# nikhilTkur/Multigrid_Nikhil_C-

Hardware: AMD Instinct MI355X
Metric: fine_grid_stencil_updates_per_sec (higher is better)
Workload: dtype f64

## Files before the change

### multigrid_nikhil_c-_amd/csrc/mgx.hip

```cpp

#include "../../include/mgx.h"
#include "mgx_bottom.hpp"
#include "mgx_kernels.hpp"
#include "mgx_launch.hpp"
#include "mgx_var.hpp"
#include "mgx_galerkin.hpp"
#include "mgx_opdep.hpp"
#include "mgx_cheby.hpp"
#include "mgx_line.hpp"
#include "mgx_small.hpp"
#include "mgx_krylov.hpp"
#include "mgx_dist_plan.hpp"

#include <chrono>
#include <unistd.h>
#include <cmath>
#include <cstdio>
#include <cstdlib>
#include <cstring>
#include <string>
#include <vector>

namespace {

using namespace mgx;

thread_local std::string g_create_error;

void log_runtime_libs(const char* where)
{
    if (env_int("MGX_LOG_RUNTIME_LIBS", 0) == 0) return;
    char buf[8192];
    if (mgx_runtime_libs(buf, sizeof buf) >= 0)
        std::fprintf(stderr, "[mgx] runtime libraries mapped at %s (pid %d):\n%s", where, (int)getpid(), buf);
}

struct Level {
    int L = 0, N = 0, rows = 0;
    long pitch = 0;
    size_t bytes = 0;
    bool f64 = true;
    void *u = nullptr, *b = nullptr, *tmp = nullptr, *r = nullptr;
    void* A[9] = {};
    void* J[9] = {};
    void* wt[8] = {nullptr, nullptr, nullptr, nullptr, nullptr, nullptr, nullptr, nullptr};
    bool nine = false;
// ... 197 lines not shown
    if (l.r) return MGX_OK;
    if (hipMalloc(&l.r, l.bytes) != hipSuccess) return s->fail(MGX_ERR_ALLOC, "hipMalloc failed for residual array");
    HIPCHK(s, hipMemsetAsync(l.r, 0, l.bytes, s->stream));
    return MGX_OK;
}

bool level_ok(const mgx_solver* s, int level)
{
    return level >= s->cfg.coarsest_level && level <= s->cfg.finest_level;
}

int copy_in(mgx_solver* s, Level& l, void* dst_grid, const void* src, size_t count)
{
    const size_t n = (size_t)l.N - 1;
    if (count != n * n) return s->fail(MGX_ERR_INVALID, "vector length must be n*n with n = 2^level - 1");
    const size_t es = l.esize();
    char* d = reinterpret_cast<char*>(dst_grid) + ((size_t)l.pitch + 1) * es;
    HIPCHK(s, hipMemcpy2DAsync(d, (size_t)l.pitch * es, src, n * es, n * es, n, hipMemcpyHostToDevice, s->stream));
    HIPCHK(s, hipStreamSynchronize(s->stream));
    return MGX_OK;
}

int copy_out(mgx_solver* s, Level& l, const void* src_grid, void* dst, size_t count)
{
    const size_t n = (size_t)l.N - 1;
    if (count != n * n) return s->fail(MGX_ERR_INVALID, "vector length must be n*n with n = 2^level - 1");
    const size_t es = l.esize();
    const char* p = reinterpret_cast<const char*>(src_grid) + ((size_t)l.pitch + 1) * es;
    HIPCHK(s, hipMemcpy2DAsync(dst, n * es, p, (size_t)l.pitch * es, n * es, n, hipMemcpyDeviceToHost, s->stream));
    HIPCHK(s, hipStreamSynchronize(s->stream));
    return MGX_OK;
}

inline bool tile_level(const mgx_solver* s, const Level& l) { return s->fuse.tile_max_n > 0 && l.N <= s->fuse.tile_max_n; }

BlockReq level_req(const mgx_solver* s, const Level& l, int mu, bool pre, int post, bool zero_in, int rpc)
{
    BlockReq q{s->cfg.smoother, l.f64, l.N, 0, l.rows, 1, l.N, mu, pre, post, zero_in};
    q.tile_points = (long)(s->fuse.tile_max_n - 1) * s->fuse.tile_max_n;
    q.rpc = rpc;
    return q;
}

int var_alloc_level(mgx_solver* s, Level& l)
{
    for (int q = 0; q < (l.nine ? 9 : 5); ++q)
        for (void** p : {&l.A[q], &l.J[q]}) {
            if (hipMalloc(p, l.bytes) != hipSuccess)
                return s->fail(MGX_ERR_ALLOC, q < 5 ? "hipMalloc failed for the operator's coefficient arrays"
                                                    : "hipMalloc failed for the nine-point operator's corner arrays");
            HIPCHK(s, hipMemsetAsync(*p, 0, l.bytes, s->stream));
        }
    return MGX_OK;
}

void gj_invert(mgx_solver* s, int NN)
{
    for (int k = 0; k < NN; ++k) {
        hipLaunchKernelGGL(k_gj_prow, dim3((NN + 255) / 256), dim3(256), 0, s->stream, s->var_M, s->var_inv, s->var_pm, s->var_pi, NN, k);
        hipLaunchKernelGGL(k_gj_elim, dim3(NN), dim3(256), 0, s->stream, s->var_M, s->var_inv, s->var_pm, s->var_pi, NN, k);
    }
}

void drop_graphs(mgx_solver* s)
{
    for (auto& g : s->graphs) if (g.exec) (void)hipGraphExecDestroy(g.exec);
// ... 876 lines not shown
    if (var && (cfg->dtype == MGX_DTYPE_MIXED || cfg->smoother == MGX_SMOOTHER_RBGS || cfg->arith != MGX_ARITH_SEPARATE || cfg->n_gpus > 1)) {
        g_create_error = cheby ? "MGX_SMOOTHER_CHEBYSHEV: dtype F64 or F32, arith SEPARATE, one GPU"
                       : galerkin ? "MGX_OPERATOR_GALERKIN: dtype F64 or F32, Jacobi or Chebyshev, arith SEPARATE, one GPU"
                                  : "MGX_OPERATOR_STENCIL5: dtype F64 or F32, Jacobi (MF:75-96) or Chebyshev, arith SEPARATE, one GPU";
        return MGX_ERR_INVALID;
    }
    if (galerkin && cfg->restrict_mode >= MGX_RESTRICT_INJECT) {
        g_create_error = "MGX_OPERATOR_GALERKIN: restrict_mode CONSISTENT or FW16 (R A P needs R = c P^T; injection has no variational meaning)";
        return MGX_ERR_INVALID;
    }
    if (cfg->restrict_mode >= MGX_RESTRICT_INJECT && (cfg->n_gpus > 1 || cfg->dtype == MGX_DTYPE_MIXED)) {
        g_create_error = "injection restriction (MF:122-130): single-GPU handles of dtype F64 or F32";
        return MGX_ERR_INVALID;
    }
    if (cfg->n_gpus > 1) return mgx_create_rank(cfg, -1, 1, nullptr, nullptr, out);
    log_runtime_libs("mgx_create");
    int ndev = 0;
    if (hipGetDeviceCount(&ndev) != hipSuccess || ndev <= 0 || cfg->device < 0 || cfg->device >= ndev) {
        g_create_error = "no usable HIP device (libmgx has no CPU fallback)";
        return MGX_ERR_NO_DEVICE;
    }
    if (hipSetDevice(cfg->device) != hipSuccess) { g_create_error = "hipSetDevice failed"; return MGX_ERR_HIP; }

    mgx_solver* s = new (std::nothrow) mgx_solver();
    if (!s) { g_create_error = "out of host memory"; return MGX_ERR_ALLOC; }
    s->cfg = *cfg;
    s->mixed = (cfg->dtype == MGX_DTYPE_MIXED);
    s->var = var;
    s->galerkin = galerkin;
    s->work_f64 = (cfg->dtype == MGX_DTYPE_F64);
    s->rows_per_chunk = env_int("MGX_ROWS", 0);
    s->fuse = fuse_cfg();
    s->fuse.arith = cfg->arith;
    s->fold = env_int("MGX_FOLD", 1);
    s->use_zero_in = env_int("MGX_ZERO_IN", 1);
    s->use_graph = env_int("MGX_GRAPH", 1);
    s->small_visit = env_int("MGX_SMALL_VISIT", 1);
    s->line_dirs = cfg->smoother == MGX_SMOOTHER_LINE_X ? 1 : cfg->smoother == MGX_SMOOTHER_LINE_Y ? 2 : cfg->smoother == MGX_SMOOTHER_LINE_ALT ? 3 : 0;
    int rc = MGX_OK;
    auto bail = [&](int code) { g_create_error = s->err; mgx_destroy(s); return code; };
    if (hipStreamCreate(&s->stream) != hipSuccess) { s->err = "hipStreamCreate failed"; return bail(MGX_ERR_HIP); }
    s->lv.resize(cfg->finest_level + 1);
    for (int l = cfg->coarsest_level; l <= cfg->finest_level; ++l)
        if ((rc = alloc_level(s, s->lv[l], l, s->work_f64)) != MGX_OK) return bail(rc);
    if (s->mixed && (rc = alloc_level(s, s->fine64, cfg->finest_level, true)) != MGX_OK) return bail(rc);
    if (var || cfg->restrict_mode >= MGX_RESTRICT_INJECT) {
        for (int l = cfg->coarsest_level + 1; l <= cfg->finest_level; ++l)
            if ((rc = ensure_r(s, s->lv[l])) != MGX_OK) return bail(rc);
    }
    if (galerkin && s->small_visit) {
        if (small_visit_prepare<double>() != hipSuccess || small_visit_prepare<float>() != hipSuccess) {
            s->err = "hipFuncSetAttribute failed for k_small_visit";
            return bail(MGX_ERR_HIP);
        }
    }
    if (var) {
        for (int l = cfg->coarsest_level; l <= cfg->finest_level; ++l) {
            s->lv[l].nine = galerkin && l < cfg->finest_level;
            if ((rc = var_alloc_level(s, s->lv[l])) != MGX_OK) return bail(rc);
            if (cheby) {
                Level& lv = s->lv[l];
                if (hipMalloc(&lv.cheb, lv.bytes) != hipSuccess) { s->err = "hipMalloc failed for the Chebyshev direction array"; return bail(MGX_ERR_ALLOC); }
                if (hipMemsetAsync(lv.cheb, 0, lv.bytes, s->stream) != hipSuccess) { s->err = "hipMemsetAsync failed"; return bail(MGX_ERR_HIP); }
            }
            if (line) {
                Level& lv = s->lv[l];
                lv.line_R = line_chunk_rows(lv.N, env_int("MGX_LINE_CHUNK", 0));
                std::vector<void**> arrays;
                for (int d = 0; d < 2; ++d)
                    if (s->line_dirs & (1 << d)) { arrays.push_back(&lv.line_m[d]); arrays.push_back(&lv.line_g[d]); }
                if ((s->line_dirs & 2) && line_chunks(lv.N, lv.line_R) > 1) { arrays.push_back(&lv.line_hf); arrays.push_back(&lv.line_hb); }
                for (void** p : arrays) {
                    if (hipMalloc(p, lv.bytes) != hipSuccess) { s->err = "hipMalloc failed for the line smoother's factor arrays"; return bail(MGX_ERR_ALLOC); }
                    if (hipMemsetAsync(*p, 0, lv.bytes, s->stream) != hipSuccess) { s->err = "hipMemsetAsync failed"; return bail(MGX_ERR_HIP); }
                }
            }
        }
        if (line && hipMalloc(&s->line_flag, sizeof(int)) != hipSuccess) { s->err = "hipMalloc failed for the line smoother's breakdown flag"; return bail(MGX_ERR_ALLOC); }
        if (cfg->bottom == MGX_BOTTOM_EXACT) {
            const size_t NN = (size_t)((1 << cfg->coarsest_level) - 1) * ((1 << cfg->coarsest_level) - 1);
            if (hipMalloc(&s->var_M, NN * NN * sizeof(double)) != hipSuccess || hipMalloc(&s->var_inv, NN * NN * sizeof(double)) != hipSuccess ||
                hipMalloc(&s->var_pm, NN * sizeof(double)) != hipSuccess || hipMalloc(&s->var_pi, NN * sizeof(double)) != hipSuccess) {
                s->err = "allocation of the coarsest operator's dense inverse failed";
                return bail(MGX_ERR_ALLOC);
            }
        }
    }
    s->mixed_fuse = env_int("MGX_MIXED_FUSE", 1);
    if (s->mixed && !s->mixed_fuse) { (void)hipFree(s->fine64.tmp); s->fine64.tmp = nullptr; }
    {
        const int N = 1 << cfg->finest_level;
        long cap = 0;
        for (int rpc : {s->rows_per_chunk, 1}) {
            cap = std::max(cap, sumsq_blocks<double>(N, N, rpc));
            cap = std::max(cap, sumsq_blocks<float>(N, N, rpc));
        }
        if (N <= s->fuse.tile_max_n) cap = std::max(cap, (long)((N + 31) / 32) * ((N + 39) / 40));
        s->partial_cap = cap + 8;
        if (hipMalloc(&s->partial, s->partial_cap * sizeof(double)) != hipSuccess ||
            hipMalloc(&s->sum_dev, sizeof(double)) != hipSuccess ||
            hipHostMalloc(&s->sum_host, sizeof(double)) != hipSuccess) {
            s->err = "allocation of reduction buffers failed";
            return bail(MGX_ERR_ALLOC);
        }
    }
    if (cfg->bottom == MGX_BOTTOM_EXACT && !var) {
        if (s->bottom.init((1 << cfg->coarsest_level) - 1) != hipSuccess) {
            s->err = "bottom solver allocation failed";
            return bail(MGX_ERR_ALLOC);
        }
    }
    if (hipStreamSynchronize(s->stream) != hipSuccess) { s->err = "device initialisation failed"; return bail(MGX_ERR_HIP); }
    *out = s;
    return MGX_OK;
}

int mgx_destroy(mgx_handle s)
{
    if (!s) return MGX_OK;
    if (s->dist) { dist_free(s->dist); s->dist = nullptr; }
    if (s->stream) (void)hipStreamSynchronize(s->stream);
    for (auto& l : s->lv) free_level(l);
    free_level(s->fine64);
    s->bottom.destroy();
    if (s->partial) (void)hipFree(s->partial);
    if (s->sum_dev) (void)hipFree(s->sum_dev);
    if (s->line_flag) (void)hipFree(s->line_flag);
    if (s->sum_host) (void)hipHostFree(s->sum_host);
    for (double* p : {s->var_M, s->var_inv, s->var_pm, s->var_pi}) if (p) (void)hipFree(p);
    s->kry.free();
// ... 690 lines not shown
    if (result_in_tmp) *result_in_tmp = flips & 1;
    return hipGetLastError() == hipSuccess ? MGX_OK : MGX_ERR_HIP;
}

int mgx_slab_jacobi(const mgx_slab* s, void* u, const void* b, void* tmp, int row_lo, int row_hi, int mu,
                    double omega, int shrink, int* result_in_tmp, void* stream)
{
    return slab_smooth(MGX_SMOOTHER_JACOBI, s, u, b, tmp, row_lo, row_hi, mu, omega, shrink, result_in_tmp, stream);
}

int mgx_slab_rbgs(const mgx_slab* s, void* u, const void* b, void* tmp, int row_lo, int row_hi, int mu,
                  int shrink, int* result_in_tmp, void* stream)
{
    return slab_smooth(MGX_SMOOTHER_RBGS, s, u, b, tmp, row_lo, row_hi, mu, 1.0, shrink, result_in_tmp, stream);
}

int mgx_slab_cycle(const mgx_slab* f, void* u, const void* b, void* tmp, int row_lo, int row_hi, int mu, double omega,
                   int smoother, const mgx_slab* c, const void* coarse_e, void* coarse_b, int crow_lo, int crow_hi,
                   int restrict_mode, int zero_in, double* scratch, double* sum_dev, int* result_in_tmp, void* stream)
{
    if (zero_in && coarse_e) return MGX_ERR_INVALID;
    if (smoother != MGX_SMOOTHER_JACOBI && smoother != MGX_SMOOTHER_RBGS) return MGX_ERR_INVALID;
    if (restrict_mode != MGX_RESTRICT_CONSISTENT && restrict_mode != MGX_RESTRICT_FW16) return MGX_ERR_INVALID;
    if (coarse_b && !((std::max(row_lo + f->row0, 1)) & 1)) return MGX_ERR_INVALID;
    if (slab_check(f) || !u || !b || !tmp || mu < 1 || mu > 64 || row_hi <= row_lo) return MGX_ERR_INVALID;
    if ((coarse_e || coarse_b) && (slab_check(c) || c->level != f->level - 1 || c->dtype != f->dtype)) return MGX_ERR_INVALID;
    if (coarse_b && sum_dev) return MGX_ERR_INVALID;
    if (sum_dev && !scratch) return MGX_ERR_INVALID;
    if (coarse_b && (crow_lo < 0 || crow_hi > c->rows || crow_hi < crow_lo)) return MGX_ERR_INVALID;
    const int N = 1 << f->level;
    if (row_lo < 0 || row_hi > f->rows || row_lo + f->row0 < 1 || row_hi + f->row0 > N) return MGX_ERR_INVALID;
    FuseCfg fc = fuse_cfg();
    fc.arith = f->arith;
    const int post = coarse_b ? 1 : (sum_dev ? 2 : 0);
    BlockReq q = slab_req(*f, smoother, row_lo, row_hi, mu, coarse_e != nullptr, post, zero_in != 0);
    q.tile_points = env_int("MGX_SLAB_TILE_POINTS", 1 << 20);
    const long pitch = level_pitch(f->level, f->dtype);
    hipStream_t st = (hipStream_t)stream;
    int flips = 0;
    const int nb = with_kernel_set(q.f64, smoother, f->arith, [&](auto k) {
        using K = decltype(k);
        using T = typename K::T;
        return fold_block<T, K::SM, K::AR>(fc, q, (T*)u, (const T*)b, (T*)tmp, pitch, omega, c, (const T*)coarse_e,
                                           (T*)coarse_b, nullptr, crow_lo, crow_hi, restrict_mode, scratch, st, &flips);
    });
    if (nb < 0) return MGX_ERR_INVALID;
    if (post == 2) hipLaunchKernelGGL(k_reduce_partials, dim3(1), dim3(kReduceThreads), 0, st, scratch, nb, sum_dev);
    if (result_in_tmp) *result_in_tmp = flips & 1;
    return hipGetLastError() == hipSuccess ? MGX_OK : MGX_ERR_HIP;
}

int mgx_slab_restrict(const mgx_slab* f, const void* u, const void* b, const mgx_slab* c, void* cb, void* zero_u,
                      int crow_lo, int crow_hi, int restrict_mode, int fused, void* stream)
{
    if (slab_check(f) || slab_check(c) || !b || !cb || (fused && !u)) return MGX_ERR_INVALID;
    if (restrict_mode != MGX_RESTRICT_CONSISTENT && restrict_mode != MGX_RESTRICT_FW16) return MGX_ERR_INVALID;
    if (c->level != f->level - 1 || c->dtype != f->dtype) return MGX_ERR_INVALID;
    const int N = 1 << f->level;
    const long pitch = level_pitch(f->level, f->dtype), cpitch = level_pitch(c->level, c->dtype);
    const int off = 2 * c->row0 - f->row0;
    const int halo = fused ? 2 : 1;
    if (crow_lo < 0 || crow_hi > c->rows || crow_lo + c->row0 < 1 || crow_hi + c->row0 > N / 2) return MGX_ERR_INVALID;
    if (crow_hi > crow_lo && (2 * crow_lo + off - halo < 0 || 2 * (crow_hi - 1) + off + halo > f->rows - 1)) return MGX_ERR_INVALID;
    const int rpc = env_int("MGX_ROWS", 0);
    if (f->dtype == MGX_DTYPE_F64)
        launch_restrict<double>((const double*)u, (const double*)b, (double*)cb, (double*)zero_u, N, pitch, cpitch,
// ... 231 lines not shown
```

### multigrid_nikhil_c-_amd/csrc/mgx_bottom.hpp

```cpp
#pragma once

#include <hip/hip_runtime.h>
#include <cmath>
#include <type_traits>
#include <vector>

#include "mgx_phase_trace.hpp"

#ifndef MGX_DST_DEEP
#define MGX_DST_DEEP 32
#endif

namespace mgx {

constexpr unsigned kDstOob = 0xFFFFFF00u;
__device__ __forceinline__ __amdgpu_buffer_rsrc_t dst_rsrc(const void* p, unsigned bytes)
{
    return __builtin_amdgcn_make_buffer_rsrc(const_cast<void*>(p), 0, (int)bytes, 0x00020000);
}
template <typename E> __device__ __forceinline__ double dst_load(__amdgpu_buffer_rsrc_t r, unsigned voff, unsigned soff)
{
    if constexpr (sizeof(E) == 8) {
        const auto t = __builtin_amdgcn_raw_buffer_load_b64(r, voff, soff, 0);
        return __hiloint2double(t[1], t[0]);
    } else {
        return (double)__int_as_float(__builtin_amdgcn_raw_buffer_load_b32(r, voff, soff, 0));
    }
}
template <typename E, int D>
__device__ __forceinline__ void dst_batch(double (&x)[D], __amdgpu_buffer_rsrc_t r, unsigned voff, unsigned rowbytes, int k0, int n)
{
    const unsigned last = (unsigned)(n - 1) * rowbytes;
    unsigned off = (unsigned)k0 * rowbytes;
#pragma unroll
    for (int q = 0; q < D; ++q, off += rowbytes) x[q] = dst_load<E>(r, voff, min(off, last));
}
template <int CNT, int D> __device__ __forceinline__ void dst_chain(double& acc, const double* m, const double (&x)[D])
{
#pragma unroll
    for (int q = 0; q < CNT; ++q) acc += m[q] * x[q];
}
template <int D> __device__ __forceinline__ void dst_chain_last(double& acc, const double* m, const double (&x)[D], int rem)
{
    if (rem == D - 1) {
        dst_chain<D - 1>(acc, m, x);
    } else {
#pragma unroll
        for (int q = 0; q < D; ++q)
            if (q < rem) acc += m[q] * x[q];
    }
}
template <int D, typename Load, typename Before, typename Stamp>
__device__ __forceinline__ double dst_dot(const double* m, int n, double (&xa)[D], Load load, Before before_last, Stamp landed)
{
    double xb[D];
    double acc = 0.0;
    int k = 0;
    for (;;) {
        if (k + D >= n) { before_last(); landed(xa[D - 1]); dst_chain_last<D>(acc, m + k, xa, n - k); break; }
        load(xb, k + D);
        landed(xa[D - 1]);
        dst_chain<D, D>(acc, m + k, xa);
        k += D;
        if (k + D >= n) { before_last(); landed(xb[D - 1]); dst_chain_last<D>(acc, m + k, xb, n - k); break; }
        load(xa, k + D);
        landed(xb[D - 1]);
        dst_chain<D, D>(acc, m + k, xb);
        k += D;
    }
    return acc;
}

template <typename T, bool FIRST>
__global__ void __launch_bounds__(256)
k_dst_pair(const double* __restrict__ S, const void* __restrict__ Xv, void* __restrict__ Ov, const double* __restrict__ s,
           int n, long gpitch)
{
    using E = std::conditional_t<FIRST, T, double>;
    __shared__ double srow[256], prow[256];
    MGX_PHASE_BEGIN();
    const int j = threadIdx.x;
    const int i = blockIdx.x;
    const bool live = j < n;
    constexpr int kDeep = MGX_DST_DEEP;
    const unsigned srb = (unsigned)n * 8u, xrb = FIRST ? (unsigned)gpitch * (unsigned)sizeof(T) : srb;
    const char* xp = static_cast<const char*>(Xv) + (FIRST ? (gpitch + 1) * (long)sizeof(T) : 0L);
    const __amdgpu_buffer_rsrc_t rs = dst_rsrc(S, (unsigned)n * srb);
    const __amdgpu_buffer_rsrc_t rx = dst_rsrc(xp, (unsigned)(n - 1) * xrb + (unsigned)n * (unsigned)sizeof(E));
    const unsigned vs = live ? (unsigned)j * 8u : kDstOob, vx = live ? (unsigned)j * (unsigned)sizeof(E) : kDstOob;
    auto landed = [&](const double& v) { MGX_PHASE_AFTER(v); (void)v; };

    const double si = dst_load<double>(rs, vs, (unsigned)i * srb);
    double ei = 0.0, ej = 0.0;
    if constexpr (FIRST) {
        const __amdgpu_buffer_rsrc_t re = dst_rsrc(s, srb);
        ei = dst_load<double>(re, live ? 0u : kDstOob, (unsigned)i * 8u);
        ej = dst_load<double>(re, vs, 0u);
    }
    double xa[kDeep], s2[kDeep];
    dst_batch<E, kDeep>(xa, rx, vx, xrb, 0, n);
    srow[j] = si;
    __syncthreads();
    const double acc = dst_dot<kDeep>(srow, n, xa, [&](double (&x)[kDeep], int k0) { dst_batch<E, kDeep>(x, rx, vx, xrb, k0, n); },
                                      [&]() { dst_batch<double, kDeep>(s2, rs, vs, srb, 0, n); }, landed);
    MGX_PHASE_AFTER(acc);
    prow[j] = acc;
    __syncthreads();
    MGX_PHASE();
    const double out = dst_dot<kDeep>(prow, n, s2, [&](double (&x)[kDeep], int k0) { dst_batch<double, kDeep>(x, rs, vs, srb, k0, n); },
                                      []() {}, landed);
    MGX_PHASE_AFTER(out);
    if (live) {
        if constexpr (FIRST) reinterpret_cast<double*>(Ov)[(long)i * n + j] = out / (ei + ej);
        else reinterpret_cast<T*>(Ov)[(long)(i + 1) * gpitch + (j + 1)] = (T)out;
    }
    MGX_PHASE_END(kPhaseDst, n | (FIRST ? 1 << 16 : 0));
}

struct BottomDST {
    int n = 0;
    double* S = nullptr;
    double* s = nullptr;
    double* w1 = nullptr;

    hipError_t init(int n_)
    {
        n = n_;
        const size_t nn = (size_t)n * n;
        std::vector<double> hS(nn), hs(n);
        const long double pi = 3.14159265358979323846264338327950288L;
        const long double norm = sqrtl(2.0L / (long double)(n + 1));
        for (int i = 0; i < n; ++i) {
            const long double a = sinl(pi * (long double)(i + 1) / (2.0L * (long double)(n + 1)));
            hs[i] = (double)(4.0L * a * a);
            for (int k = 0; k < n; ++k) {
                const long m = ((long)(i + 1) * (long)(k + 1)) % (2L * (n + 1));
                hS[(size_t)i * n + k] = (double)(norm * sinl(pi * (long double)m / (long double)(n + 1)));
            }
        }
        hipError_t e;
        if ((e = hipMalloc(&S, nn * sizeof(double))) != hipSuccess) return e;
        if ((e = hipMalloc(&s, n * sizeof(double))) != hipSuccess) return e;
        if ((e = hipMalloc(&w1, nn * sizeof(double))) != hipSuccess) return e;
        if ((e = hipMemcpy(S, hS.data(), nn * sizeof(double), hipMemcpyHostToDevice)) != hipSuccess) return e;
        if ((e = hipMemcpy(s, hs.data(), n * sizeof(double), hipMemcpyHostToDevice)) != hipSuccess) return e;
        return hipSuccess;
    }

    void destroy()
    {
        if (S) (void)hipFree(S);
        if (s) (void)hipFree(s);
        if (w1) (void)hipFree(w1);
        S = s = w1 = nullptr;
    }

    template <typename T>
    void solve(const T* b_grid, T* u_grid, long gpitch, hipStream_t st) const
    {
        const int block = (n + 63) / 64 * 64;
        hipLaunchKernelGGL((k_dst_pair<T, true>), dim3(n), dim3(block), 0, st, S, (const void*)b_grid, (void*)w1, s, n, gpitch);
        hipLaunchKernelGGL((k_dst_pair<T, false>), dim3(n), dim3(block), 0, st, S, (const void*)w1, (void*)u_grid, s, n, gpitch);
    }
};

}
```

### multigrid_nikhil_c-_amd/csrc/mgx_geom.hpp

```cpp
#pragma once

#if defined(__HIPCC__)
#define MGX_GEOM_HD __host__ __device__ __forceinline__
#else
#define MGX_GEOM_HD inline
#endif

namespace mgx {

constexpr int kGeomWavesPerBlock = 4;
constexpr int kGeomCusPerXcd = 32;
constexpr int kGeomResidentBlocks = 512;

struct CycleGeom {
    int R, Re, Rl;
    int Rf;
    int chunks, chunks_e;
    int row_last0;
    int RB, n_tall, n_short;
    long waves;
    int blocks;
};

struct CTile { int strip, r0, r1; bool active; };
// ... 215 lines not shown
        CycleGeom p;
        if (cycle_geom_paired(row_lo, row_hi, strips, extra, trip, kn, top_edge, bot_edge, &p)) return p;
    }
    bool found = false;
    for (int m = (row_hi - row_lo >= kn.min_rounds_rows ? kn.min_rounds : 1); m <= 64 && !found; ++m) {
        for (int r = trip_rows(kn.min_chunk, extra, trip, 2); r <= 204; r += trip) {
            const CycleGeom c = shaped(r);
            if (c.waves <= 2048L * m && c.blocks <= kGeomResidentBlocks * m) { g = c; found = true; break; }
        }
    }
    return g;
}

constexpr int kTileWideWaves = 8;

struct TileWideGeom {
    int He, Hx;
    int TH, TW;
    int tiles_y, tiles_x;
};

MGX_GEOM_HD TileWideGeom tile_wide_geom(int N, int row_lo, int row_hi, int He, int W, int RW)
{
    TileWideGeom g;
    g.He = He;
    g.Hx = (He + W - 1) / W * W;
    g.TH = kTileWideWaves * RW - 2 * He;
    g.TW = 64 * W - 2 * g.Hx;
    g.tiles_y = (g.TH > 0 && row_hi > row_lo) ? (row_hi - row_lo + g.TH - 1) / g.TH : 0;
    g.tiles_x = g.TW > 0 ? (N + g.TW - 1) / g.TW : 0;
    return g;
}

MGX_GEOM_HD int tile_wide_rw(int N, int short_max_n) { return N <= short_max_n ? 8 : 10; }

}
```

### multigrid_nikhil_c-_amd/csrc/mgx_kernels.hpp

```cpp
#pragma once

#include <hip/hip_runtime.h>
#include "mgx_geom.hpp"
#include "mgx_phase_trace.hpp"
#include <stdint.h>
#include <type_traits>

namespace mgx {

template <int B, int E, typename F> __device__ __forceinline__ void static_for(F&& f)
{
    if constexpr (B < E) {
        f(std::integral_constant<int, B>{});
        static_for<B + 1, E>(f);
    }
}

constexpr int kWave = 64;
constexpr int kBlock = 256;
constexpr int kWavesPerBlock = kBlock / kWave;
constexpr int kOutLanes = kWave - 2;

template <typename T> struct VecOf;
template <> struct VecOf<double> { using type = double2; static constexpr int W = 2; };
// ... 1587 lines not shown
    const int ty = blockIdx.x / tiles_x, tx = blockIdx.x - ty * tiles_x;
    const int y0 = wv * RW;
    const int gy0 = row_lo + ty * TH - He + y0;
    const int cx0 = tx * TW;
    const int gx0 = cx0 - g.Hx + W * lane;
    const bool vld = gx0 >= 0 && gx0 < N;
    const bool cu0 = vld && gx0 > 0;
    bool cu[W];
#pragma unroll
    for (int e = 0; e < W; ++e) cu[e] = e == 0 ? cu0 : vld;
    const int NC = N / 2;
    MGX_PHASE_AFTER(gx0 + gy0);

    T u[RW][W], b[RW][W];
    unsigned rowmask = 0;
#pragma unroll
    for (int i = 0; i < RW; ++i) {
        const int gy = gy0 + i;
        const bool rowok = gy > 0 && gy < N && gy >= win.row_first && gy <= win.row_last;
        if (rowok) rowmask |= 1u << i;
        const long at = (long)gy * pitch + gx0;
        V uv = vzero((V*)nullptr), bv = vzero((V*)nullptr);
        if (vld && rowok) {
            bv = *reinterpret_cast<const V*>(rhs + at);
            if (!zero_in) uv = *reinterpret_cast<const V*>(vin + at);
        }
#pragma unroll
        for (int e = 0; e < W; ++e) {
            u[i][e] = cu[e] ? vget(uv, e) : (T)0;
            b[i][e] = cu[e] ? vget(bv, e) : (T)0;
        }
    }
    if (PRE) {
        constexpr int NCR = RW / 2 + 1, NCC = W / 2 + 1;
        const int kc0 = gy0 >> 1, J = gx0 >> 1;
        T cr[NCR][NCC];
#pragma unroll
        for (int k = 0; k < NCR; ++k) {
            const int cy = kc0 + k;
            const bool ok = vld && cy >= 0 && cy <= NC && cy >= win.crow_first && cy <= win.crow_last;
            const T* ep = coarse_e + (long)cy * cpitch + J;
#pragma unroll
            for (int m = 0; m < NCC; ++m) cr[k][m] = ok ? ep[m] : (T)0;
        }
        auto correct = [&](auto parity) {
            constexpr int par = decltype(parity)::value;
#pragma unroll
            for (int i = 0; i < RW; ++i) {
                const int gy = gy0 + i;
                const bool rodd = ((par + i) & 1) != 0;
                const int kr = (par + i) >> 1;
                const bool rin = ((rowmask >> i) & 1u) && (gy >> 1) >= win.crow_first && (gy >> 1) + (rodd ? 1 : 0) <= win.crow_last;
#pragma unroll
                for (int e = 0; e < W; ++e) {
                    const bool codd = (e & 1) != 0;
                    const bool unk = cu[e] && rin;
                    const T a00 = unk ? cr[kr][e >> 1] : (T)0;
                    const T a01 = (unk && codd) ? cr[kr][(e >> 1) + 1] : (T)0;
                    const T a10 = (unk && rodd) ? cr[kr + (rodd ? 1 : 0)][e >> 1] : (T)0;
                    const T a11 = (unk && rodd && codd) ? cr[kr + (rodd ? 1 : 0)][(e >> 1) + 1] : (T)0;
                    const T ev = codd ? (T)0.5 * (a00 + a01) : a00;
                    const T od = codd ? (T)0.25 * (((a00 + a10) + a01) + a11) : (T)0.5 * (a00 + a10);
                    const T add = rodd ? od : ev;
                    u[i][e] = unk ? u[i][e] + add : u[i][e];
                }
            }
        };
// ... 252 lines not shown
```

### multigrid_nikhil_c-_amd/csrc/mgx_launch.hpp

```cpp
#pragma once

#include "../../include/mgx.h"
#include "mgx_kernels.hpp"
#include "mgx_pass_plan.hpp"

#include <algorithm>

namespace mgx {

inline long level_pitch(int level, int dtype)
{
    const long N = 1L << level;
    const long align = (dtype == MGX_DTYPE_F64) ? 32 : 64;
    return (N + 1 + align - 1) / align * align;
}

template <typename T> struct JacobiCoef { T c0, c1; };
template <typename T>
JacobiCoef<T> jacobi_coef(double omega)
{
    const T om = (T)omega;
    return {(T)(1.0 - (double)om), (T)((double)om / 4.0)};
}

// ... 154 lines not shown
            case 5: return launch_cycle_k<T, 5, PRE, POST, 0, AR>(vin, b, vout, fa, N, pitch, c0, c1, R, st);
            default: break;
        }
    }
    return -1;
}

template <int PRE_, int POST_> struct Stages { static constexpr int PRE = PRE_, POST = POST_; };
template <typename F>
int with_stages(bool pre, int post, F&& f)
{
    if (pre) return post == 2 ? f(Stages<1, 2>{}) : (post == 1 ? f(Stages<1, 1>{}) : f(Stages<1, 0>{}));
    return post == 2 ? f(Stages<0, 2>{}) : (post == 1 ? f(Stages<0, 1>{}) : f(Stages<0, 0>{}));
}

template <typename T, int SM, int PRE, int POST, int AR>
int launch_tile(const T* vin, const T* b, T* vout, const FoldArgs& fa, int N, long pitch, T c0, T c1, int levels,
                hipStream_t st)
{
    const int He = levels + tile_extra<POST>();
    const int TH = kTileSY - 2 * He, TW = kTileSX - 2 * He;
    if (TH < 8 || TW < 8) return -1;
    const int row_lo = fa.row_lo, row_hi = fa.row_hi;
    const CycleWin& win = fa.win;
    const int tiles_y = (row_hi - row_lo + TH - 1) / TH, tiles_x = (N - 1 + TW - 1) / TW;
    if (tiles_y < 1) return 0;
    const T w = (fa.restrict_mode == MGX_RESTRICT_FW16) ? (T)0.0625 : (T)0.25;
    hipLaunchKernelGGL((k_tile_smooth<T, SM, PRE, POST, AR>), dim3(tiles_y * tiles_x), dim3(kBlock), 0, st, vin, b, vout,
                       (const T*)fa.coarse_e, (T*)fa.coarse_b, (T*)fa.coarse_zero, w, fa.partial, N, pitch, fa.cpitch,
                       levels, c0, c1, tiles_x, fa.zero_in, row_lo, row_hi, win);
    return tiles_y * tiles_x;
}

template <typename T, int SM, int PRE, int POST, int AR>
int launch_tile_wide(const T* vin, const T* b, T* vout, const FoldArgs& fa, int N, long pitch, T c0, T c1, int levels,
                     int rw, hipStream_t st)
{
    if (VecOf<T>::W == 4) rw = 8;
    const int row_lo = fa.row_lo, row_hi = fa.row_hi;
    const CycleWin& win = fa.win;
    const TileWideGeom g = tile_wide_geom(N, row_lo, row_hi, levels + tile_extra<POST>(), VecOf<T>::W, rw);
    if (g.TH < 8 || g.TW < 8) return -1;
    if (g.tiles_y < 1) return 0;
    const T w = (fa.restrict_mode == MGX_RESTRICT_FW16) ? (T)0.0625 : (T)0.25;
    const dim3 grid(g.tiles_y * g.tiles_x), block(kTileWideWaves * kWave);
    if (rw == 8)
        hipLaunchKernelGGL((k_tile_wide<T, SM, PRE, POST, AR, 8>), grid, block, 0, st, vin, b, vout, (const T*)fa.coarse_e,
                           (T*)fa.coarse_b, (T*)fa.coarse_zero, w, fa.partial, N, pitch, fa.cpitch, levels, c0, c1, g.tiles_x,
                           fa.zero_in, row_lo, row_hi, win);
    else if constexpr (VecOf<T>::W == 2) {
        if (rw != 10) return -1;
        hipLaunchKernelGGL((k_tile_wide<T, SM, PRE, POST, AR, 10>), grid, block, 0, st, vin, b, vout, (const T*)fa.coarse_e,
                           (T*)fa.coarse_b, (T*)fa.coarse_zero, w, fa.partial, N, pitch, fa.cpitch, levels, c0, c1, g.tiles_x,
                           fa.zero_in, row_lo, row_hi, win);
    } else {
        return -1;
    }
    return g.tiles_y * g.tiles_x;
}

template <typename T, int SM, int AR>
int launch_tile_pass(const T* vin, const T* b, T* vout, const FoldArgs& fa, int N, long pitch, T c0, T c1, int levels,
                     int band, bool pre, int post, hipStream_t st)
{
    return with_stages(pre, post, [&](auto s) {
        using S = decltype(s);
        return band ? launch_tile_wide<T, SM, S::PRE, S::POST, AR>(vin, b, vout, fa, N, pitch, c0, c1, levels, band, st)
                    : launch_tile<T, SM, S::PRE, S::POST, AR>(vin, b, vout, fa, N, pitch, c0, c1, levels, st);
    });
}

template <typename T>
void launch_restrict(const T* v, const T* b, T* cb, T* czero, int N, long pitch, long cpitch,
                     int crow_lo, int crow_hi, int fine_row_off, int mode, bool fused, int rpc, hipStream_t st)
{
    if (crow_hi <= crow_lo) return;
    Launch g = make_launch(N, VecOf<T>::W, crow_hi - crow_lo, rpc > 0 ? (rpc + 1) / 2 : 0);
    const T w = (mode == MGX_RESTRICT_FW16) ? (T)0.0625 : (T)0.25;
    if (fused)
        hipLaunchKernelGGL((k_restrict<T, true>), dim3(g.blocks), dim3(kBlock), 0, st, v, b, cb, czero, N, pitch,
                           cpitch, crow_lo, crow_hi, fine_row_off, g.R, g.strips, g.chunks, w);
    else
        hipLaunchKernelGGL((k_restrict<T, false>), dim3(g.blocks), dim3(kBlock), 0, st, v, b, cb, czero, N, pitch,
                           cpitch, crow_lo, crow_hi, fine_row_off, g.R, g.strips, g.chunks, w);
}

template <typename T>
void launch_prolong(T* v, const T* e, int N, long pitch, long cpitch, int row_lo, int row_hi,
                    int fine_row_off, bool add, int rpc, hipStream_t st)
{
// ... 49 lines not shown
```

### multigrid_nikhil_c-_amd/csrc/mgx_pass_plan.hpp

```cpp
#pragma once

#include "../../include/mgx.h"
#include "mgx_geom.hpp"

#include <algorithm>
#include <cstdlib>
#include <vector>

namespace mgx {

inline int env_int(const char* name, int dflt)
{
    const char* s = getenv(name);
    return (s && *s) ? atoi(s) : dflt;
}

struct FuseCfg {
    int kmax; int rows; int min_n; int fold_kmax; int fold_kmax_big; int tile_max_n; int tile_k; int fold_kmax_nopost;
    int tile_wide; int tile_short_n;
    int plan_pre[8] = {0}; int n_pre = 0; int plan_post[8] = {0}; int n_post = 0; int plan_min_n = 8192;
    int arith = 0;
};

inline int fuse_rows_deep(int N, int rows)
{
    const int strips = (N / 2 + 51) / 52;
    const int cpr = std::max(1, 2048 / strips);
    for (int m = 1; m <= 64; ++m) {
        const int R = (rows + m * cpr - 1) / (m * cpr);
        if (R <= 200) return std::max(R, 16);
    }
    return 64;
}

inline bool fuse_rows_auto(const FuseCfg& fc, int N, int K, bool f64)
{
    return fc.rows <= 0 && K >= (f64 ? 8 : 10) && N >= 2048;
}

inline int shallow_big_n() { static const int n = env_int("MGX_SHALLOW_BIG_N", 8192); return n; }
inline int shallow_mid_rows() { static const int r = env_int("MGX_SHALLOW_ROWS_MID", 48); return r; }

inline int fuse_rows(const FuseCfg& fc, int N, int K, bool f64 = true, int rows = 0)
{
    if (fc.rows > 0) return fc.rows;
    if (K <= 2) {
        static const int big2 = env_int("MGX_SHALLOW2_ROWS_BIG", 96);
        return N >= shallow_big_n() ? big2 : (N >= 4096 ? shallow_mid_rows() : 8);
    }
    if (K <= 4) {
        static const int big = env_int("MGX_SHALLOW_ROWS_BIG", 96);
        return N >= shallow_big_n() ? big : (N >= 4096 ? shallow_mid_rows() : 16);
    }
    if (f64 && K >= 8 && N >= 2048) return fuse_rows_deep(N, rows > 0 ? rows : N - 1);
    int R = N / 128;
    if (R < 8) R = 8;
    if (R > (f64 ? 64 : 32)) R = f64 ? 64 : 32;
    return R;
}

inline FuseCfg fuse_cfg()
{
    FuseCfg f;
    f.kmax = env_int("MGX_FUSE", 10);
    if (f.kmax < 1) f.kmax = 1;
    if (f.kmax > 10) f.kmax = 10;
    f.rows = env_int("MGX_FUSE_ROWS", 0);
    if (f.rows < 0) f.rows = 0;
    f.min_n = std::max(64, env_int("MGX_FUSE_MIN_N", 256));
    f.fold_kmax = std::max(1, std::min(f.kmax, env_int("MGX_FOLD_KMAX", 10)));
    f.fold_kmax_big = std::max(1, std::min(f.kmax, env_int("MGX_FOLD_KMAX_BIG", 10)));
    f.tile_wide = std::max(0, std::min(2, env_int("MGX_TILE_WIDE", 1)));
    f.tile_short_n = env_int("MGX_TILE_SHORT_N", 512);
    f.tile_max_n = std::max(0, env_int("MGX_TILE_MAX_N", 1024));
    f.tile_k = std::max(2, std::min(10, env_int("MGX_TILE_K", 10)));
    f.fold_kmax_nopost = std::max(1, std::min(f.kmax, env_int("MGX_FOLD_KMAX_NOPOST", 10)));
    auto parse = [](const char* name, int* out) {
        const char* v = std::getenv(name);
        int n = 0;
        while (v && *v && n < 8) {
            char* end = nullptr;
            const long k = std::strtol(v, &end, 10);
            if (end == v || k < 1 || k > 10) return 0;
            out[n++] = (int)k;
            v = (*end == ',') ? end + 1 : end;
            if (*end && *end != ',') return 0;
        }
        return n;
    };
    f.n_pre = parse("MGX_PLAN_PRE", f.plan_pre);
    f.n_post = parse("MGX_PLAN_POST", f.plan_post);
    f.plan_min_n = env_int("MGX_PLAN_MIN_N", 8192);
    return f;
}

inline bool cycle_k_supported(int K, bool rbgs, bool f64, int post, bool pre, int arith)
{
    if (K == 10) return !(pre && post == 1) && !(rbgs && post == 1) && !(!f64 && pre && post == 2) && !(!f64 && post == 1 && arith == 0);
    if (K == 8 && !f64 && !pre && post != 0) return false;
    return rbgs ? (K == 2 || K == 4 || K == 6 || K == 8) : (K >= 1 && K <= 8 && K != 7);
}

inline bool fused_k_supported(int K, bool rbgs)
{
    return K == 2 || K == 4 || K == 6 || K == 8 || K == 10 || (!rbgs && (K == 3 || K == 5));
}

inline int tile_band(const FuseCfg& fc, int N, bool f64)
{
    return (fc.tile_wide >= (f64 ? 1 : 2)) ? tile_wide_rw(N, fc.tile_short_n) : 0;
}

constexpr double kFuseRate64[11] = {0, 1.00, 1.80, 2.45, 3.16, 3.81, 4.80, 0, 5.60, 0, 5.63};
constexpr double kFuseRate32[11] = {0, 1.00, 1.67, 2.38, 3.10, 3.77, 4.26, 0, 4.98, 0, 4.67};
constexpr double kFuseRateGS64[11] = {0, 1.00, 1.81, 2.50, 3.19, 3.12, 0, 0, 0, 0, 0};
constexpr double kFuseRateGS32[11] = {0, 1.00, 1.79, 2.20, 2.87, 2.69, 0, 0, 0, 0, 0};

inline double fold_pass_cost(int K, bool rbgs, int post, bool f64, int arith)
{
    if (!cycle_k_supported(K, rbgs, f64, post, false, arith)) return -1.0;
    if (rbgs) return K <= 4 ? 1.0 : (K == 6 ? 1.1 : (K == 8 ? 1.3 : 2.4));
    if (K <= 5) return 1.0;
    if (!f64) return K == 6 ? 1.34 : (K == 8 ? 1.53 : 1.75);
    if (K == 6) return 1.05;
    if (K == 8) return 1.12;
    return 1.46;
}

template <typename Cost>
std::vector<int> split_sweeps(int mu, int smax, double launch, double eps, Cost cost)
{
    std::vector<double> best(mu + 1, 1e300);
    std::vector<int> pick(mu + 1, 1);
    best[0] = 0.0;
    for (int m = 1; m <= mu; ++m)
        for (int k = 1; k <= std::min(m, smax); ++k) {
            const double c = cost(k, m);
            if (c < 0.0) continue;
            const double t = best[m - k] + c + launch;
            if (t < best[m] - eps) { best[m] = t; pick[m] = k; }
        }
    std::vector<int> parts;
    for (int m = mu; m > 0; m -= pick[m]) parts.push_back(pick[m]);
// ... 14 lines not shown
    bool pre; int post;
    bool zero_in;
    int lo, hi;
    int R;
};

struct BlockReq {
    int smoother = MGX_SMOOTHER_JACOBI; bool f64 = true;
    int N = 0, row0 = 0, rows = 0;
    int row_lo = 0, row_hi = 0;
    int mu = 0;
    bool pre = false;
    int post = 0;
    bool zero_in = false;
    bool widen = true;
    bool strict = false;
    long tile_points = 0;
    int rpc = 0;
};

inline bool fold_plan(const FuseCfg& fc, const BlockReq& q, std::vector<Pass>* plan)
{
    plan->clear();
    const bool rbgs = (q.smoother == MGX_SMOOTHER_RBGS);
    const int per = rbgs ? 2 : 1, N = q.N, mu = q.mu;
    const int first = 1 - q.row0, last = N - q.row0;
    {
        const int lo = std::max(std::max(q.row_lo, first), 1), hi = std::min(std::min(q.row_hi, last), q.rows - 1);
        const bool whole = q.row_lo <= first && q.row_hi >= last;
        if (fc.tile_max_n > 0 && hi > lo && (long)(hi - lo) * N <= q.tile_points && (per * mu <= fc.tile_k || whole)) {
            const int smax = std::max(1, fc.tile_k / per), np = (mu + smax - 1) / smax;
            for (int p = 0; p < np; ++p) {
                const int sw = mu / np + (p < mu % np ? 1 : 0);
                plan->push_back({PASS_TILE, per * sw, q.pre && p == 0, p == np - 1 ? q.post : 0, q.zero_in && p == 0,
                                 lo + q.row0, hi + q.row0, tile_band(fc, N, q.f64)});
            }
            return true;
        }
    }
    const bool staged = q.pre || q.post != 0;
    const bool fuse = fc.kmax > per && N >= fc.min_n && (q.row_hi - q.row_lo) >= 64 && mu <= 64;
    std::vector<int> parts;
    if (!staged) {
        const double* rate = rbgs ? (q.f64 ? kFuseRateGS64 : kFuseRateGS32) : (q.f64 ? kFuseRate64 : kFuseRate32);
        if (fuse)
            parts = split_sweeps(mu, std::max(1, std::min(fc.kmax, 10) / per), 0.02, 0.0,
                                 [&](int k, int) { return rate[k] > 0.0 ? (double)k / rate[k] : -1.0; });
        else
            parts.assign(std::max(mu, 0), 1);
    } else {
        const int* forced = nullptr;
        int nf = 0;
        if (!q.pre && q.post == 1) { forced = fc.plan_pre; nf = fc.n_pre; }
        else if (q.pre) { forced = fc.plan_post; nf = fc.n_post; }
        if (nf > 0 && N >= fc.plan_min_n) {
            int sum = 0;
            bool ok = true;
            for (int i = 0; i < nf; ++i) {
                sum += forced[i];
                const int K = per * forced[i];
                const bool folded = (i == 0 && q.pre) || (i == nf - 1 && q.post != 0);
                const int Q = (i == nf - 1) ? q.post : 0;
                ok = ok && K <= 10 && (folded ? cycle_k_supported(K, rbgs, q.f64, Q, q.pre && i == 0, fc.arith) : (K != 7 && K != 9 && (!rbgs || K % 2 == 0)));
            }
            if (ok && sum == mu) parts.assign(forced, forced + nf);
        }
        if (parts.empty()) {
            int kcap = N >= 8192 ? fc.fold_kmax_big : fc.fold_kmax;
// ... 42 lines not shown
```

Before: 1128 billion.

## Pick tile-wide row band by CU count; add multi-row DST bottom kernel

For f64 tiled passes, the row-band width of the wide tile kernel is now chosen from a larger set of instantiated values (4–10). The choice picks the first width whose tile grid fits within the device's compute-unit count, with the aim of spreading small levels across more CUs instead of using a fixed 8 or 10. A knob also lets the DST bottom solver process several rows per block, but its default stays at one row, so that path is inactive. A PRE coarse-register sizing fix covers odd row widths. The trade-off is more kernel instantiations, and smaller bands add halo overhead.

```diff
diff --git a/multigrid_nikhil_c-_amd/csrc/mgx.hip b/multigrid_nikhil_c-_amd/csrc/mgx.hip
--- a/multigrid_nikhil_c-_amd/csrc/mgx.hip
+++ b/multigrid_nikhil_c-_amd/csrc/mgx.hip
@@ -12,6 +12,7 @@
 #include "mgx_krylov.hpp"
 #include "mgx_dist_plan.hpp"
 
+#include <atomic>
 #include <chrono>
 #include <unistd.h>
 #include <cmath>
@@ -275,6 +276,17 @@
     return MGX_OK;
 }
 
+inline int device_cus()
+{
+    static std::atomic<int> known[64];
+    int dev = 0, n = 0;
+    if (hipGetDevice(&dev) != hipSuccess || dev < 0 || dev >= 64) return 0;
+    if ((n = known[dev].load(std::memory_order_relaxed)) > 0) return n;
+    if (hipDeviceGetAttribute(&n, hipDeviceAttributeMultiprocessorCount, dev) != hipSuccess || n < 0) n = 0;
+    known[dev].store(n, std::memory_order_relaxed);
+    return n;
+}
+
 inline bool tile_level(const mgx_solver* s, const Level& l) { return s->fuse.tile_max_n > 0 && l.N <= s->fuse.tile_max_n; }
 
 BlockReq level_req(const mgx_solver* s, const Level& l, int mu, bool pre, int post, bool zero_in, int rpc)
@@ -1217,6 +1229,7 @@
     s->rows_per_chunk = env_int("MGX_ROWS", 0);
     s->fuse = fuse_cfg();
     s->fuse.arith = cfg->arith;
+    s->fuse.cus = device_cus();
     s->fold = env_int("MGX_FOLD", 1);
     s->use_zero_in = env_int("MGX_ZERO_IN", 1);
     s->use_graph = env_int("MGX_GRAPH", 1);
@@ -1280,7 +1293,7 @@
             cap = std::max(cap, sumsq_blocks<double>(N, N, rpc));
             cap = std::max(cap, sumsq_blocks<float>(N, N, rpc));
         }
-        if (N <= s->fuse.tile_max_n) cap = std::max(cap, (long)((N + 31) / 32) * ((N + 39) / 40));
+        if (N <= s->fuse.tile_max_n) cap = std::max(cap, (long)((N + kTileWideMinTH - 1) / kTileWideMinTH) * ((N + 39) / 40));
         s->partial_cap = cap + 8;
         if (hipMalloc(&s->partial, s->partial_cap * sizeof(double)) != hipSuccess ||
             hipMalloc(&s->sum_dev, sizeof(double)) != hipSuccess ||
@@ -2037,6 +2050,7 @@
     if (row_lo < 0 || row_hi > f->rows || row_lo + f->row0 < 1 || row_hi + f->row0 > N) return MGX_ERR_INVALID;
     FuseCfg fc = fuse_cfg();
     fc.arith = f->arith;
+    fc.cus = device_cus();
     const int post = coarse_b ? 1 : (sum_dev ? 2 : 0);
     BlockReq q = slab_req(*f, smoother, row_lo, row_hi, mu, coarse_e != nullptr, post, zero_in != 0);
     q.tile_points = env_int("MGX_SLAB_TILE_POINTS", 1 << 20);
diff --git a/multigrid_nikhil_c-_amd/csrc/mgx_bottom.hpp b/multigrid_nikhil_c-_amd/csrc/mgx_bottom.hpp
--- a/multigrid_nikhil_c-_amd/csrc/mgx_bottom.hpp
+++ b/multigrid_nikhil_c-_amd/csrc/mgx_bottom.hpp
@@ -2,6 +2,7 @@
 
 #include <hip/hip_runtime.h>
 #include <cmath>
+#include <cstdlib>
 #include <type_traits>
 #include <vector>
 
@@ -35,52 +36,59 @@
 #pragma unroll
     for (int q = 0; q < D; ++q, off += rowbytes) x[q] = dst_load<E>(r, voff, min(off, last));
 }
-template <int CNT, int D> __device__ __forceinline__ void dst_chain(double& acc, const double* m, const double (&x)[D])
-{
-#pragma unroll
-    for (int q = 0; q < CNT; ++q) acc += m[q] * x[q];
-}
-template <int D> __device__ __forceinline__ void dst_chain_last(double& acc, const double* m, const double (&x)[D], int rem)
+constexpr int kDstRow = 256;
+template <int CNT, int ROWS, int D> __device__ __forceinline__ void dst_chain(double (&acc)[ROWS], const double* m, const double (&x)[D])
+{
+#pragma unroll
+    for (int q = 0; q < CNT; ++q)
+#pragma unroll
+        for (int r = 0; r < ROWS; ++r) acc[r] += m[r * kDstRow + q] * x[q];
+}
+template <int ROWS, int D> __device__ __forceinline__ void dst_chain_last(double (&acc)[ROWS], const double* m, const double (&x)[D], int rem)
 {
     if (rem == D - 1) {
         dst_chain<D - 1>(acc, m, x);
     } else {
 #pragma unroll
         for (int q = 0; q < D; ++q)
-            if (q < rem) acc += m[q] * x[q];
-    }
-}
-template <int D, typename Load, typename Before, typename Stamp>
-__device__ __forceinline__ double dst_dot(const double* m, int n, double (&xa)[D], Load load, Before before_last, Stamp landed)
+            if (q < rem) {
+#pragma unroll
+                for (int r = 0; r < ROWS; ++r) acc[r] += m[r * kDstRow + q] * x[q];
+            }
+    }
+}
+template <int D, int ROWS, typename Load, typename Before, typename Stamp>
+__device__ __forceinline__ void dst_dot(double (&acc)[ROWS], const double* m, int n, double (&xa)[D], Load load, Before before_last, Stamp landed)
 {
     double xb[D];
-    double acc = 0.0;
+#pragma unroll
+    for (int r = 0; r < ROWS; ++r) acc[r] = 0.0;
     int k = 0;
     for (;;) {
-        if (k + D >= n) { before_last(); landed(xa[D - 1]); dst_chain_last<D>(acc, m + k, xa, n - k); break; }
+        if (k + D >= n) { before_last(); landed(xa[D - 1]); dst_chain_last(acc, m + k, xa, n - k); break; }
         load(xb, k + D);
         landed(xa[D - 1]);
-        dst_chain<D, D>(acc, m + k, xa);
+        dst_chain<D>(acc, m + k, xa);
         k += D;
-        if (k + D >= n) { before_last(); landed(xb[D - 1]); dst_chain_last<D>(acc, m + k, xb, n - k); break; }
+        if (k + D >= n) { before_last(); landed(xb[D - 1]); dst_chain_last(acc, m + k, xb, n - k); break; }
         load(xa, k + D);
         landed(xb[D - 1]);
-        dst_chain<D, D>(acc, m + k, xb);
+        dst_chain<D>(acc, m + k, xb);
         k += D;
     }
-    return acc;
-}
-
-template <typename T, bool FIRST>
+}
+
+template <typename T, bool FIRST, int ROWS>
 __global__ void __launch_bounds__(256)
 k_dst_pair(const double* __restrict__ S, const void* __restrict__ Xv, void* __restrict__ Ov, const double* __restrict__ s,
            int n, long gpitch)
 {
     using E = std::conditional_t<FIRST, T, double>;
-    __shared__ double srow[256], prow[256];
+    __shared__ double srow[ROWS * kDstRow], prow[ROWS * kDstRow];
     MGX_PHASE_BEGIN();
     const int j = threadIdx.x;
-    const int i = blockIdx.x;
+    const int i0 = blockIdx.x * ROWS;
+    const int nr = min(ROWS, n - i0);
     const bool live = j < n;
     constexpr int kDeep = MGX_DST_DEEP;
     const unsigned srb = (unsigned)n * 8u, xrb = FIRST ? (unsigned)gpitch * (unsigned)sizeof(T) : srb;
@@ -90,31 +98,51 @@
     const unsigned vs = live ? (unsigned)j * 8u : kDstOob, vx = live ? (unsigned)j * (unsigned)sizeof(E) : kDstOob;
     auto landed = [&](const double& v) { MGX_PHASE_AFTER(v); (void)v; };
 
-    const double si = dst_load<double>(rs, vs, (unsigned)i * srb);
-    double ei = 0.0, ej = 0.0;
-    if constexpr (FIRST) {
-        const __amdgpu_buffer_rsrc_t re = dst_rsrc(s, srb);
-        ei = dst_load<double>(re, live ? 0u : kDstOob, (unsigned)i * 8u);
-        ej = dst_load<double>(re, vs, 0u);
-    }
+    double si[ROWS];
+    double ei[ROWS], ej = 0.0;
+#pragma unroll
+    for (int r = 0; r < ROWS; ++r) {
+        const unsigned i = (unsigned)min(i0 + r, n - 1);
+        si[r] = dst_load<double>(rs, vs, i * srb);
+        ei[r] = 0.0;
+        if constexpr (FIRST) ei[r] = dst_load<double>(dst_rsrc(s, srb), live ? 0u : kDstOob, i * 8u);
+    }
+    if constexpr (FIRST) ej = dst_load<double>(dst_rsrc(s, srb), vs, 0u);
     double xa[kDeep], s2[kDeep];
     dst_batch<E, kDeep>(xa, rx, vx, xrb, 0, n);
-    srow[j] = si;
+#pragma unroll
+    for (int r = 0; r < ROWS; ++r) srow[r * kDstRow + j] = si[r];
     __syncthreads();
-    const double acc = dst_dot<kDeep>(srow, n, xa, [&](double (&x)[kDeep], int k0) { dst_batch<E, kDeep>(x, rx, vx, xrb, k0, n); },
-                                      [&]() { dst_batch<double, kDeep>(s2, rs, vs, srb, 0, n); }, landed);
-    MGX_PHASE_AFTER(acc);
-    prow[j] = acc;
+    double acc[ROWS], out[ROWS];
+    dst_dot<kDeep>(acc, srow, n, xa, [&](double (&x)[kDeep], int k0) { dst_batch<E, kDeep>(x, rx, vx, xrb, k0, n); },
+                   [&]() { dst_batch<double, kDeep>(s2, rs, vs, srb, 0, n); }, landed);
+    MGX_PHASE_AFTER(acc[ROWS - 1]);
+#pragma unroll
+    for (int r = 0; r < ROWS; ++r) prow[r * kDstRow + j] = acc[r];
     __syncthreads();
     MGX_PHASE();
-    const double out = dst_dot<kDeep>(prow, n, s2, [&](double (&x)[kDeep], int k0) { dst_batch<double, kDeep>(x, rs, vs, srb, k0, n); },
-                                      []() {}, landed);
-    MGX_PHASE_AFTER(out);
+    dst_dot<kDeep>(out, prow, n, s2, [&](double (&x)[kDeep], int k0) { dst_batch<double, kDeep>(x, rs, vs, srb, k0, n); },
+                   []() {}, landed);
+    MGX_PHASE_AFTER(out[ROWS - 1]);
     if (live) {
-        if constexpr (FIRST) reinterpret_cast<double*>(Ov)[(long)i * n + j] = out / (ei + ej);
-        else reinterpret_cast<T*>(Ov)[(long)(i + 1) * gpitch + (j + 1)] = (T)out;
-    }
-    MGX_PHASE_END(kPhaseDst, n | (FIRST ? 1 << 16 : 0));
+#pragma unroll
+        for (int r = 0; r < ROWS; ++r) {
+            const int i = i0 + r;
+            if (r < nr) {
+                if constexpr (FIRST) reinterpret_cast<double*>(Ov)[(long)i * n + j] = out[r] / (ei[r] + ej);
+                else reinterpret_cast<T*>(Ov)[(long)(i + 1) * gpitch + (j + 1)] = (T)out[r];
+            }
+        }
+    }
+    MGX_PHASE_END(kPhaseDst, n | (FIRST ? 1 << 16 : 0) | (ROWS << 20));
+}
+
+constexpr int kDstRowsDefault = 1;
+inline int dst_rows_knob()
+{
+    const char* e = getenv("MGX_DST_ROWS");
+    const int v = (e && *e) ? atoi(e) : 0;
+    return (v == 1 || v == 2 || v == 4) ? v : kDstRowsDefault;
 }
 
 struct BottomDST {
@@ -122,10 +150,12 @@
     double* S = nullptr;
     double* s = nullptr;
     double* w1 = nullptr;
+    int rows = kDstRowsDefault;
 
     hipError_t init(int n_)
     {
         n = n_;
+        rows = dst_rows_knob();
         const size_t nn = (size_t)n * n;
         std::vector<double> hS(nn), hs(n);
         const long double pi = 3.14159265358979323846264338327950288L;
@@ -155,12 +185,21 @@
         S = s = w1 = nullptr;
     }
 
+    template <typename T, int ROWS>
+    void solve_rows(const T* b_grid, T* u_grid, long gpitch, hipStream_t st) const
+    {
+        const int block = (n + 63) / 64 * 64;
+        const dim3 grid((n + ROWS - 1) / ROWS);
+        hipLaunchKernelGGL((k_dst_pair<T, true, ROWS>), grid, dim3(block), 0, st, S, (const void*)b_grid, (void*)w1, s, n, gpitch);
+        hipLaunchKernelGGL((k_dst_pair<T, false, ROWS>), grid, dim3(block), 0, st, S, (const void*)w1, (void*)u_grid, s, n, gpitch);
+    }
+
     template <typename T>
     void solve(const T* b_grid, T* u_grid, long gpitch, hipStream_t st) const
     {
-        const int block = (n + 63) / 64 * 64;
-        hipLaunchKernelGGL((k_dst_pair<T, true>), dim3(n), dim3(block), 0, st, S, (const void*)b_grid, (void*)w1, s, n, gpitch);
-        hipLaunchKernelGGL((k_dst_pair<T, false>), dim3(n), dim3(block), 0, st, S, (const void*)w1, (void*)u_grid, s, n, gpitch);
+        if (rows == 4) solve_rows<T, 4>(b_grid, u_grid, gpitch, st);
+        else if (rows == 2) solve_rows<T, 2>(b_grid, u_grid, gpitch, st);
+        else solve_rows<T, 1>(b_grid, u_grid, gpitch, st);
     }
 };
 
diff --git a/multigrid_nikhil_c-_amd/csrc/mgx_geom.hpp b/multigrid_nikhil_c-_amd/csrc/mgx_geom.hpp
--- a/multigrid_nikhil_c-_amd/csrc/mgx_geom.hpp
+++ b/multigrid_nikhil_c-_amd/csrc/mgx_geom.hpp
@@ -271,6 +271,34 @@
     return g;
 }
 
-MGX_GEOM_HD int tile_wide_rw(int N, int short_max_n) { return N <= short_max_n ? 8 : 10; }
-
-}
+constexpr int kTileWideRws[] = {4, 5, 6, 8, 9, 10};
+constexpr int kTileWideNumRws = (int)(sizeof(kTileWideRws) / sizeof(kTileWideRws[0]));
+constexpr int kTileWideMinTH = 8, kTileWideMinTW = 8;
+
+MGX_GEOM_HD bool tile_wide_rw_inst(int rw)
+{
+    for (int i = 0; i < kTileWideNumRws; ++i)
+        if (kTileWideRws[i] == rw) return true;
+    return false;
+}
+
+MGX_GEOM_HD bool tile_wide_fits(const TileWideGeom& g) { return g.TH >= kTileWideMinTH && g.TW >= kTileWideMinTW; }
+
+MGX_GEOM_HD int tile_wide_rw_fixed(int N, int short_max_n) { return N <= short_max_n ? 8 : 10; }
+
+MGX_GEOM_HD int tile_wide_rw(int N, int row_lo, int row_hi, int He, int W, int cus, int short_max_n, int knob)
+{
+    if (W != 2) return 8;
+    const int fixed = tile_wide_rw_fixed(N, short_max_n);
+    if (knob < 0) return fixed;
+    if (knob > 0 && tile_wide_rw_inst(knob) && tile_wide_fits(tile_wide_geom(N, row_lo, row_hi, He, W, knob))) return knob;
+    if (cus > 0) {
+        for (int i = 0; i < kTileWideNumRws; ++i) {
+            const TileWideGeom g = tile_wide_geom(N, row_lo, row_hi, He, W, kTileWideRws[i]);
+            if (tile_wide_fits(g) && (long)g.tiles_y * g.tiles_x <= cus) return kTileWideRws[i];
+        }
+    }
+    return tile_wide_fits(tile_wide_geom(N, row_lo, row_hi, He, W, fixed)) ? fixed : kTileWideRws[kTileWideNumRws - 1];
+}
+
+}
diff --git a/multigrid_nikhil_c-_amd/csrc/mgx_kernels.hpp b/multigrid_nikhil_c-_amd/csrc/mgx_kernels.hpp
--- a/multigrid_nikhil_c-_amd/csrc/mgx_kernels.hpp
+++ b/multigrid_nikhil_c-_amd/csrc/mgx_kernels.hpp
@@ -1643,7 +1643,7 @@
         }
     }
     if (PRE) {
-        constexpr int NCR = RW / 2 + 1, NCC = W / 2 + 1;
+        constexpr int NCR = (RW + 1) / 2 + 1, NCC = W / 2 + 1;
         const int kc0 = gy0 >> 1, J = gx0 >> 1;
         T cr[NCR][NCC];
 #pragma unroll
diff --git a/multigrid_nikhil_c-_amd/csrc/mgx_launch.hpp b/multigrid_nikhil_c-_amd/csrc/mgx_launch.hpp
--- a/multigrid_nikhil_c-_amd/csrc/mgx_launch.hpp
+++ b/multigrid_nikhil_c-_amd/csrc/mgx_launch.hpp
@@ -210,30 +210,38 @@
     return tiles_y * tiles_x;
 }
 
+template <typename T, int SM, int PRE, int POST, int AR, int RW>
+void launch_tile_wide_rw(const T* vin, const T* b, T* vout, const FoldArgs& fa, int N, long pitch, T c0, T c1, int levels,
+                         const TileWideGeom& g, hipStream_t st)
+{
+    const T w = (fa.restrict_mode == MGX_RESTRICT_FW16) ? (T)0.0625 : (T)0.25;
+    hipLaunchKernelGGL((k_tile_wide<T, SM, PRE, POST, AR, RW>), dim3(g.tiles_y * g.tiles_x), dim3(kTileWideWaves * kWave), 0, st,
+                       vin, b, vout, (const T*)fa.coarse_e, (T*)fa.coarse_b, (T*)fa.coarse_zero, w, fa.partial, N, pitch,
+                       fa.cpitch, levels, c0, c1, g.tiles_x, fa.zero_in, fa.row_lo, fa.row_hi, fa.win);
+}
+
 template <typename T, int SM, int PRE, int POST, int AR>
 int launch_tile_wide(const T* vin, const T* b, T* vout, const FoldArgs& fa, int N, long pitch, T c0, T c1, int levels,
                      int rw, hipStream_t st)
 {
     if (VecOf<T>::W == 4) rw = 8;
-    const int row_lo = fa.row_lo, row_hi = fa.row_hi;
-    const CycleWin& win = fa.win;
-    const TileWideGeom g = tile_wide_geom(N, row_lo, row_hi, levels + tile_extra<POST>(), VecOf<T>::W, rw);
-    if (g.TH < 8 || g.TW < 8) return -1;
+    const TileWideGeom g = tile_wide_geom(N, fa.row_lo, fa.row_hi, levels + tile_extra<POST>(), VecOf<T>::W, rw);
+    if (!tile_wide_fits(g)) return -1;
     if (g.tiles_y < 1) return 0;
-    const T w = (fa.restrict_mode == MGX_RESTRICT_FW16) ? (T)0.0625 : (T)0.25;
-    const dim3 grid(g.tiles_y * g.tiles_x), block(kTileWideWaves * kWave);
-    if (rw == 8)
-        hipLaunchKernelGGL((k_tile_wide<T, SM, PRE, POST, AR, 8>), grid, block, 0, st, vin, b, vout, (const T*)fa.coarse_e,
-                           (T*)fa.coarse_b, (T*)fa.coarse_zero, w, fa.partial, N, pitch, fa.cpitch, levels, c0, c1, g.tiles_x,
-                           fa.zero_in, row_lo, row_hi, win);
-    else if constexpr (VecOf<T>::W == 2) {
-        if (rw != 10) return -1;
-        hipLaunchKernelGGL((k_tile_wide<T, SM, PRE, POST, AR, 10>), grid, block, 0, st, vin, b, vout, (const T*)fa.coarse_e,
-                           (T*)fa.coarse_b, (T*)fa.coarse_zero, w, fa.partial, N, pitch, fa.cpitch, levels, c0, c1, g.tiles_x,
-                           fa.zero_in, row_lo, row_hi, win);
+#define MGX_TILE_RW_CASE(RW_) \
+    case RW_: launch_tile_wide_rw<T, SM, PRE, POST, AR, RW_>(vin, b, vout, fa, N, pitch, c0, c1, levels, g, st); break
+    if constexpr (VecOf<T>::W == 2) {
+        switch (rw) {
+            MGX_TILE_RW_CASE(4); MGX_TILE_RW_CASE(5); MGX_TILE_RW_CASE(6); MGX_TILE_RW_CASE(8); MGX_TILE_RW_CASE(9); MGX_TILE_RW_CASE(10);
+            default: return -1;
+        }
     } else {
-        return -1;
-    }
+        switch (rw) {
+            MGX_TILE_RW_CASE(8);
+            default: return -1;
+        }
+    }
+#undef MGX_TILE_RW_CASE
     return g.tiles_y * g.tiles_x;
 }
 
diff --git a/multigrid_nikhil_c-_amd/csrc/mgx_pass_plan.hpp b/multigrid_nikhil_c-_amd/csrc/mgx_pass_plan.hpp
--- a/multigrid_nikhil_c-_amd/csrc/mgx_pass_plan.hpp
+++ b/multigrid_nikhil_c-_amd/csrc/mgx_pass_plan.hpp
@@ -20,6 +20,7 @@
     int tile_wide; int tile_short_n;
     int plan_pre[8] = {0}; int n_pre = 0; int plan_post[8] = {0}; int n_post = 0; int plan_min_n = 8192;
     int arith = 0;
+    int tile_rw = 0; int cus = 0;
 };
 
 inline int fuse_rows_deep(int N, int rows)
@@ -72,6 +73,7 @@
     f.fold_kmax_big = std::max(1, std::min(f.kmax, env_int("MGX_FOLD_KMAX_BIG", 10)));
     f.tile_wide = std::max(0, std::min(2, env_int("MGX_TILE_WIDE", 1)));
     f.tile_short_n = env_int("MGX_TILE_SHORT_N", 512);
+    f.tile_rw = env_int("MGX_TILE_RW", 0);
     f.tile_max_n = std::max(0, env_int("MGX_TILE_MAX_N", 1024));
     f.tile_k = std::max(2, std::min(10, env_int("MGX_TILE_K", 10)));
     f.fold_kmax_nopost = std::max(1, std::min(f.kmax, env_int("MGX_FOLD_KMAX_NOPOST", 10)));
@@ -106,9 +108,11 @@
     return K == 2 || K == 4 || K == 6 || K == 8 || K == 10 || (!rbgs && (K == 3 || K == 5));
 }
 
-inline int tile_band(const FuseCfg& fc, int N, bool f64)
-{
-    return (fc.tile_wide >= (f64 ? 1 : 2)) ? tile_wide_rw(N, fc.tile_short_n) : 0;
+inline int tile_band(const FuseCfg& fc, int N, bool f64, int lo, int hi, int K, int post)
+{
+    if (fc.tile_wide < (f64 ? 1 : 2)) return 0;
+    const int He = K + (post == 1 ? 2 : (post == 2 ? 1 : 0));
+    return tile_wide_rw(N, lo, hi, He, f64 ? 2 : 4, fc.cus, fc.tile_short_n, fc.tile_rw);
 }
 
 constexpr double kFuseRate64[11] = {0, 1.00, 1.80, 2.45, 3.16, 3.81, 4.80, 0, 5.60, 0, 5.63};
@@ -189,8 +193,9 @@
             const int smax = std::max(1, fc.tile_k / per), np = (mu + smax - 1) / smax;
             for (int p = 0; p < np; ++p) {
                 const int sw = mu / np + (p < mu % np ? 1 : 0);
-                plan->push_back({PASS_TILE, per * sw, q.pre && p == 0, p == np - 1 ? q.post : 0, q.zero_in && p == 0,
-                                 lo + q.row0, hi + q.row0, tile_band(fc, N, q.f64)});
+                const int K = per * sw, Q = p == np - 1 ? q.post : 0;
+                plan->push_back({PASS_TILE, K, q.pre && p == 0, Q, q.zero_in && p == 0, lo + q.row0, hi + q.row0,
+                                 tile_band(fc, N, q.f64, lo + q.row0, hi + q.row0, K, Q)});
             }
             return true;
         }
```

New measurement: 1139 billion, median of 6. Within noise of the previous version (+1.0%).
